# codgodtao/TMDiff

Hardware: AMD Instinct MI355X
Metric: UNet denoise-steps/sec (8-ch 64x64, batch 32) (higher is better)
Workload: dtype f32; 1 GPU; BASELINE configs[1]: batch-32 8-ch 64x64 tiles, DDPM p_sample steps of the T=1000 cosine schedule, channel_multiplier [32,64,128,256], full UNet forward (both branches) + fused DDPM update per step; batch_per_gpu=32, parallelism=batch-parallel x1, weights=key-hashed random init, text_embedding=fixed synthetic 768-d

## Files before the change

include/tmdiff_hip.h:

```cpp
#ifndef TMDIFF_HIP_H
#define TMDIFF_HIP_H

#include <stddef.h>
#include <stdint.h>

#ifdef __cplusplus
extern "C" {
#endif

#define TMDIFF_ABI_VERSION 6

#define TMDIFF_OK 0
#define TMDIFF_E_INVALID (-1)
#define TMDIFF_E_UNSUPPORTED (-2)
#define TMDIFF_E_LAUNCH (-3)

typedef void* tmdiff_stream_t;

int tmdiff_version(void);
const char* tmdiff_last_error_string(void);

typedef struct tmdiff_conv3d_desc {
  int32_t B, N, H, W;
  int32_t Cin, Cout;
// ... 15 lines not shown
  float out_scale;
  float* y;
  float* y2;
  const float* y2_shift;
  const float* y2_scale;
  int32_t y2_shift_stride, y2_scale_stride;
  int32_t y2_act;
  int32_t y2_bf16;
  int32_t x_bf16;
  void* splitk_ws;
  int64_t splitk_ws_bytes;
  uint64_t drop_seed;
  float drop_p;
  const uint64_t* drop_seed_dev;
  const float* rc_x;
  const float* rc_w;
  int32_t rc_cin;
  float* y_ll;
  float* y_hi[3];
  float* xp_out;
  const float* xp_shift;
  int32_t xp_shift_stride, xp_act;
  int32_t y2_s2d;
} tmdiff_conv3d_desc;

int tmdiff_conv3d_pack_weights(const float* w, float* packed, int32_t Cout, int32_t Cin, int32_t ksize,
                               int32_t groups, int32_t mode, tmdiff_stream_t stream);
typedef struct tmdiff_pack_entry {
  const float* w;
  float* packed_fwd;
  float* packed_dgrad;
  int32_t Cout, Cin, ksize, groups;
} tmdiff_pack_entry;
int32_t tmdiff_conv3d_pack_weights_multi_chunks(int32_t Cout, int32_t Cin, int32_t groups, int32_t* n_type_a);
int tmdiff_conv3d_pack_weights_multi(const tmdiff_pack_entry* entries_dev, const int32_t* chunk_tensor_dev,
                                     const int32_t* chunk_index_dev, int32_t n_chunks, tmdiff_stream_t stream);
int tmdiff_conv3d_fwd(const tmdiff_conv3d_desc* d, tmdiff_stream_t stream);
int tmdiff_conv3d_fwd_xp_supported(const tmdiff_conv3d_desc* d);
size_t tmdiff_conv3d_fwd_splitk_workspace_bytes(const tmdiff_conv3d_desc* d);

int tmdiff_conv3d_fwd_staged_supported(const tmdiff_conv3d_desc* d);
size_t tmdiff_conv3d_fwd_staged_workspace_bytes(const tmdiff_conv3d_desc* d);
int tmdiff_conv3d_fwd_staged(const tmdiff_conv3d_desc* d, void* workspace, tmdiff_stream_t stream);

int tmdiff_conv3d_ll_supported(const tmdiff_conv3d_desc* d);
size_t tmdiff_conv3d_ll_splitk_workspace_bytes(const tmdiff_conv3d_desc* d);
// ... 4 lines not shown

int tmdiff_conv3d_wino_supported(const tmdiff_conv3d_desc* d);
int32_t tmdiff_conv3d_wino_planes(int32_t N);
int64_t tmdiff_conv3d_wino_blocks(const tmdiff_conv3d_desc* d);
size_t tmdiff_conv3d_wino_workspace_bytes(const tmdiff_conv3d_desc* d);
size_t tmdiff_conv3d_wino_packed_bytes(int32_t Cout, int32_t Cin, int32_t groups, int32_t planes);
int tmdiff_conv3d_wino_pack_weights(const float* w, float* packed, int32_t Cout, int32_t Cin, int32_t groups,
                                    int32_t mode, int32_t planes, tmdiff_stream_t stream);
typedef struct tmdiff_wino_pack_entry {
  const float* w;
  float* packed;
  int32_t Cout, Cin, groups, mode, planes, reserved;
} tmdiff_wino_pack_entry;
int32_t tmdiff_conv3d_wino_pack_weights_multi_chunk(void);
int tmdiff_conv3d_wino_pack_weights_multi(const tmdiff_wino_pack_entry* entries_dev, const int32_t* chunk_tensor_dev,
                                          const int32_t* chunk_index_dev, int32_t n_chunks, tmdiff_stream_t stream);
int tmdiff_conv3d_wino_fwd(const tmdiff_conv3d_desc* d, void* workspace, tmdiff_stream_t stream);
int tmdiff_conv3d_wino_fwd_stage(const tmdiff_conv3d_desc* d, void* workspace, int32_t stage, tmdiff_stream_t stream);
int tmdiff_conv3d_wino_fwd_xp(const tmdiff_conv3d_desc* d, void* workspace, int32_t stage, float* xp_out, tmdiff_stream_t stream);
int tmdiff_conv3d_wino_fwd_planes(const tmdiff_conv3d_desc* d, void* workspace, int32_t stage, float* xp_out, int32_t planes,
                                  tmdiff_stream_t stream);

int tmdiff_conv3d_wf_supported(const tmdiff_conv3d_desc* d);
int64_t tmdiff_conv3d_wf_blocks(const tmdiff_conv3d_desc* d);
size_t tmdiff_conv3d_wf_splitk_workspace_bytes(const tmdiff_conv3d_desc* d);
size_t tmdiff_conv3d_wf_workspace_bytes(const tmdiff_conv3d_desc* d);
int32_t tmdiff_conv3d_wf_plan(int32_t B, int32_t Cin, int32_t Cout, int32_t N, int32_t H, int32_t W, int32_t groups, int32_t llm,
                              int64_t* tiles);
int tmdiff_conv3d_wf_fwd(const tmdiff_conv3d_desc* d, void* workspace, tmdiff_stream_t stream);
int tmdiff_conv3d_wfll_supported(const tmdiff_conv3d_desc* d);
size_t tmdiff_conv3d_wfll_packed_bytes(int32_t Cout, int32_t Cin);
int tmdiff_conv3d_wfll_pack_weights(const float* w, float* packed, int32_t Cout, int32_t Cin, float ll_scale,
                                    tmdiff_stream_t stream);
size_t tmdiff_conv3d_wfll_splitk_workspace_bytes(const tmdiff_conv3d_desc* d);
int tmdiff_conv3d_wfll_fwd(const tmdiff_conv3d_desc* d, float ll_scale, tmdiff_stream_t stream);

size_t tmdiff_conv3d_packed_bf16_bytes(int32_t Cout, int32_t Cin, int32_t ksize, int32_t groups);
int tmdiff_conv3d_pack_weights_bf16(const float* w, void* packed, int32_t Cout, int32_t Cin, int32_t ksize,
                                    int32_t groups, tmdiff_stream_t stream);
int tmdiff_conv3d_pack_weights_bf16_dgrad(const float* w, void* packed, int32_t Cout, int32_t Cin, int32_t ksize,
                                          int32_t groups, tmdiff_stream_t stream);
size_t tmdiff_conv3d_bf16_workspace_bytes(const tmdiff_conv3d_desc* d);
int tmdiff_conv3d_fwd_bf16(const tmdiff_conv3d_desc* d, void* workspace, tmdiff_stream_t stream);


int tmdiff_conv3d_prologue_fwd(const tmdiff_conv3d_desc* d, float* xp, tmdiff_stream_t stream);
// ... 259 lines not shown
```

tmdiff_amd/_lib.py:

```python
import ctypes as C
import os

_HERE = os.path.dirname(os.path.abspath(__file__))
LIB_PATH = os.environ.get("TMDIFF_HIP_LIB") or os.path.join(_HERE, "libtmdiff_hip.so")

c_float_p = C.POINTER(C.c_float)
vp = C.c_void_p


class Conv3dDesc(C.Structure):
    _fields_ = [
        ("B", C.c_int32), ("N", C.c_int32), ("H", C.c_int32), ("W", C.c_int32),
        ("Cin", C.c_int32), ("Cout", C.c_int32),
        ("groups", C.c_int32), ("ksize", C.c_int32), ("nseg", C.c_int32),
        ("seg_c", C.c_int32 * 3),
        ("seg_x", vp * 3),
        ("w_packed", vp), ("bias", vp), ("bias_scale", C.c_float),
        ("in_shift", vp), ("in_scale", vp), ("in_shift_stride", C.c_int32), ("in_scale_stride", C.c_int32),
        ("in_mask", vp), ("in_act", C.c_int32),
        ("residual", vp), ("out_scale", C.c_float),
        ("y", vp),
        ("y2", vp), ("y2_shift", vp), ("y2_scale", vp), ("y2_shift_stride", C.c_int32), ("y2_scale_stride", C.c_int32),
        ("y2_act", C.c_int32), ("y2_bf16", C.c_int32), ("x_bf16", C.c_int32),
        ("splitk_ws", vp), ("splitk_ws_bytes", C.c_int64),
        ("drop_seed", C.c_uint64), ("drop_p", C.c_float), ("drop_seed_dev", vp), ("rc_x", vp), ("rc_w", vp), ("rc_cin", C.c_int32), ("y_ll", vp), ("y_hi", vp * 3), ("xp_out", vp), ("xp_shift", vp), ("xp_shift_stride", C.c_int32), ("xp_act", C.c_int32),
        ("y2_s2d", C.c_int32),
    ]


SIGNATURES = {
    "tmdiff_version": (C.c_int, []),
    "tmdiff_last_error_string": (C.c_char_p, []),
    "tmdiff_conv3d_pack_weights": (C.c_int, [vp, vp, C.c_int32, C.c_int32, C.c_int32, C.c_int32, C.c_int32, vp]),
    "tmdiff_conv3d_pack_weights_multi_chunks": (C.c_int32, [C.c_int32, C.c_int32, C.c_int32, C.POINTER(C.c_int32)]),
    "tmdiff_conv3d_pack_weights_multi": (C.c_int, [vp, vp, vp, C.c_int32, vp]),
    "tmdiff_conv3d_fwd": (C.c_int, [C.POINTER(Conv3dDesc), vp]),
    "tmdiff_conv3d_fwd_splitk_workspace_bytes": (C.c_size_t, [C.POINTER(Conv3dDesc)]),
    "tmdiff_conv3d_fwd_xp_supported": (C.c_int, [C.POINTER(Conv3dDesc)]),
    "tmdiff_conv3d_fwd_staged_supported": (C.c_int, [C.POINTER(Conv3dDesc)]),
    "tmdiff_conv3d_fwd_staged_workspace_bytes": (C.c_size_t, [C.POINTER(Conv3dDesc)]),
    "tmdiff_conv3d_fwd_staged": (C.c_int, [C.POINTER(Conv3dDesc), vp, vp]),
    "tmdiff_conv3d_wino_supported": (C.c_int, [C.POINTER(Conv3dDesc)]),
    "tmdiff_conv3d_wino_blocks": (C.c_int64, [C.POINTER(Conv3dDesc)]),
    "tmdiff_conv3d_wino_workspace_bytes": (C.c_size_t, [C.POINTER(Conv3dDesc)]),
    "tmdiff_conv3d_wino_planes": (C.c_int32, [C.c_int32]),
    "tmdiff_conv3d_wino_packed_bytes": (C.c_size_t, [C.c_int32, C.c_int32, C.c_int32, C.c_int32]),
    "tmdiff_conv3d_wino_pack_weights": (C.c_int, [vp, vp, C.c_int32, C.c_int32, C.c_int32, C.c_int32, C.c_int32, vp]),
    "tmdiff_conv3d_wino_pack_weights_multi_chunk": (C.c_int32, []),
    "tmdiff_conv3d_wino_pack_weights_multi": (C.c_int, [vp, vp, vp, C.c_int32, vp]),
    "tmdiff_conv3d_wf_supported": (C.c_int, [C.POINTER(Conv3dDesc)]),
    "tmdiff_conv3d_wf_blocks": (C.c_int64, [C.POINTER(Conv3dDesc)]),
    "tmdiff_conv3d_wf_workspace_bytes": (C.c_size_t, [C.POINTER(Conv3dDesc)]),
    "tmdiff_conv3d_wf_splitk_workspace_bytes": (C.c_size_t, [C.POINTER(Conv3dDesc)]),
    "tmdiff_conv3d_wf_fwd": (C.c_int, [C.POINTER(Conv3dDesc), vp, vp]),
    "tmdiff_conv3d_wino_fwd": (C.c_int, [C.POINTER(Conv3dDesc), vp, vp]),
    "tmdiff_conv3d_wino_fwd_planes": (C.c_int, [C.POINTER(Conv3dDesc), vp, C.c_int32, vp, C.c_int32, vp]),
    "tmdiff_conv3d_wino_fwd_xp": (C.c_int, [C.POINTER(Conv3dDesc), vp, C.c_int32, vp, vp]),
    "tmdiff_conv3d_wino_fwd_stage": (C.c_int, [C.POINTER(Conv3dDesc), vp, C.c_int32, vp]),
    "tmdiff_conv3d_prologue_fwd": (C.c_int, [C.POINTER(Conv3dDesc), vp, vp]),
    "tmdiff_conv3d_ll_supported": (C.c_int, [C.POINTER(Conv3dDesc)]),
    "tmdiff_conv3d_ll_splitk_workspace_bytes": (C.c_size_t, [C.POINTER(Conv3dDesc)]),
    "tmdiff_conv3d_ll_packed_bytes": (C.c_size_t, [C.c_int32, C.c_int32]),
    "tmdiff_conv3d_ll_pack_weights": (C.c_int, [vp, vp, C.c_int32, C.c_int32, C.c_float, vp]),
    "tmdiff_conv3d_ll_fwd": (C.c_int, [C.POINTER(Conv3dDesc), C.c_float, vp]),
    "tmdiff_conv3d_packed_bf16_bytes": (C.c_size_t, [C.c_int32, C.c_int32, C.c_int32, C.c_int32]),
    "tmdiff_conv3d_pack_weights_bf16": (C.c_int, [vp, vp, C.c_int32, C.c_int32, C.c_int32, C.c_int32, vp]),
    "tmdiff_conv3d_bf16_workspace_bytes": (C.c_size_t, [C.POINTER(Conv3dDesc)]),
    "tmdiff_conv3d_fwd_bf16": (C.c_int, [C.POINTER(Conv3dDesc), vp, vp]),
    "tmdiff_conv3d_wgrad_workspace_bytes": (C.c_size_t, [C.POINTER(Conv3dDesc)]),
    "tmdiff_conv3d_wgrad": (C.c_int, [C.POINTER(Conv3dDesc), vp, vp, vp, vp]),
    "tmdiff_conv3d_wgrad_bias": (C.c_int, [C.POINTER(Conv3dDesc), vp, vp, vp, vp, vp]),
    "tmdiff_conv3d_wf_plan": (C.c_int32, [C.c_int32] * 8 + [C.POINTER(C.c_int64)]),
    "tmdiff_conv3d_wfll_supported": (C.c_int, [C.POINTER(Conv3dDesc)]),
    "tmdiff_conv3d_wfll_packed_bytes": (C.c_size_t, [C.c_int32, C.c_int32]),
# ... 163 lines not shown
```

tmdiff_amd/csrc/conv3d_wf.hip:

```cpp
#include <type_traits>

#include "common.h"
#include "epilogue.h"

#ifndef TMDIFF_WF_ABLATE
#define TMDIFF_WF_ABLATE 0
#endif
#ifndef TMDIFF_WF_STAMPS
#define TMDIFF_WF_STAMPS 0
#endif

namespace {

using namespace tmdiff;

using f32x4 = __attribute__((ext_vector_type(4))) float;
using f32x2 = __attribute__((ext_vector_type(2))) float;

struct WfArgs {
  int B, N, H, W;
  int Cin, Cout, cin_g, cout_g, groups;
  const float* x;
  const float* xgrp[3];
  int grouped_segs;
  const float* wp;
  const float* bias;
  float bias_scale;
  const float* residual;
  float out_scale;
  float* y;
  float* y2;
  const float* y2_shift;
  const float* y2_scale;
  int y2_shift_stride, y2_scale_stride, y2_act;
  int y2_s2d;
  int tiles_h, tiles_w, tiles_co;
  unsigned total_blocks;
  int vec4;
  int ksplit, split_chunks;
  float* part;
  unsigned long long* stamps;
  int stagger;
  unsigned first_round;
  float* yll;
  float* yhi[3];
  const float* rc_x;
  const float* rc_w;
  int rc_cin;
};

#if defined(__HIP_DEVICE_COMPILE__)
using KArgs = const WfArgs __attribute__((address_space(4)))*;
__device__ __forceinline__ KArgs kargs() {
  KArgs k = (KArgs)__builtin_amdgcn_kernarg_segment_ptr();
  asm volatile("" : "+s"(k));
  return k;
}
#else
using KArgs = const WfArgs*;
__device__ __forceinline__ KArgs kargs() { return nullptr; }
#endif

template <class T>
// ... 170 lines not shown
  using G = GeoF<TT, TH, TW, PAIR, LLM>;
  constexpr int NP = G::NP, MO = G::MO, KC = G::KC, CO = G::CO, NS = G::NS, HH = G::HH, RQ = G::RQ, PW = G::PW;
  constexpr int W_TAPS = G::W_TAPS;
  __shared__ __attribute__((aligned(16))) float lds[2 * G::STAGE + G::RAW_FLOATS];
  float* const st0 = lds;
  float* const st1 = lds + G::STAGE;
  float* const raw = lds + 2 * G::STAGE;
  static_assert(2 * G::STAGE + G::RAW_FLOATS >= 4 * 1024, "the epilogue borrows 4 KB of LDS per wave");

  const int tid = threadIdx.x;
  const int lane = tid & 63, wv = __builtin_amdgcn_readfirstlane(tid >> 6);
  const int l31 = lane & 31, khalf = lane >> 5;
#if TMDIFF_WF_STAMPS
  unsigned long long stamp_t[6];
  const unsigned long long stamp_c0 = __builtin_amdgcn_s_memtime();
  stamp_t[0] = __builtin_amdgcn_s_memrealtime();
#define WF_STAMP(i) stamp_t[i] = __builtin_amdgcn_s_memrealtime()
#else
#define WF_STAMP(i)
#endif
  stagger_start(a.stagger, a.first_round);
  WF_STAMP(1);

  unsigned id = xcd_remap(blockIdx.x, a.total_blocks);
  const int split = take(id, a.ksplit);
  const int co_tile = take(id, a.tiles_co);
  const int tw_i = take(id, a.tiles_w);
  const int th_i = take(id, a.tiles_h);
  const int g = __builtin_amdgcn_readfirstlane(id % a.groups);
  const int b = __builtin_amdgcn_readfirstlane(id / a.groups) * (PAIR ? 2 : 1);
  const bool pimg_ok = !PAIR || b + 1 < a.B;
  const int h0 = th_i * TH, w0 = tw_i * TW;
  const int co0 = co_tile * CO;
  const int hw = a.H * a.W;
  const long plane = (long)a.N * hw;
  const int nchunks = a.split_chunks;
  const float* xg = (a.grouped_segs ? (g == 0 ? a.xgrp[0] : (g == 1 ? a.xgrp[1] : a.xgrp[2])) + (long)b * a.cin_g * plane
                                    : a.x + ((long)b * a.Cin + (long)g * a.cin_g) * plane) + (long)split * nchunks * KC * plane;
  const float* wg = a.wp + ((long)g * a.cin_g + (long)split * nchunks * KC) * W_TAPS * a.cout_g + co0;

  const long xbs = PAIR && pimg_ok ? (long)(a.grouped_segs ? a.cin_g : a.Cin) * plane : 0;
  const unsigned xbytes = (unsigned)((xbs + KC * plane) * 4), wbytes = (unsigned)(KC * W_TAPS * a.cout_g * 4);
  const int xq = lane % G::REG_QUADS, xsub = lane / G::REG_QUADS;
  unsigned xlane_off;
  if constexpr (PAIR) {
    const int img = (xq % RQ) >> 1;
    xlane_off = (lane < G::PLANES && (img == 0 || pimg_ok)) ? (unsigned)((img * xbs + (xq / RQ) * hw + 4 * (xq & 1)) * 4) : buf::kOutside;
  } else {
    const int xwq = w0 - 4 + 4 * (xq % RQ);
    xlane_off = (lane < G::PLANES && xwq >= 0 && xwq < a.W) ? (unsigned)(((xq / RQ) * hw + xwq) * 4) : buf::kOutside;
  }
  auto issue_raw = [&](auto kc_, int c) __attribute__((always_inline)) {
    constexpr int k = decltype(kc_)::value;
    const int p = wv + 4 * k;
    if (G::XP % 4 == 0 || p < G::XP) {
      const buf::rsrc r = buf::make(xg + (long)c * KC * plane, xbytes);
      const int region = p * G::RPP + (G::RPP > 1 ? xsub : 0);
      const int kc = region / HH, row = region - kc * HH;
      const int h = h0 - 1 + row;
      const bool ok = h >= 0 && h < a.H && region < G::NREG;
      const unsigned lo = opaque(xlane_off);
      const unsigned voff = ok ? lo + (unsigned)((kc * (int)plane + h * a.W) * 4) : buf::kOutside;
// ... 218 lines not shown
  }
#undef WF_EPI2
#if TMDIFF_WF_STAMPS
  WF_STAMP(4);
  __builtin_amdgcn_s_waitcnt(0);
  WF_STAMP(5);
  if (a.stamps && lane == 0) {
    unsigned long long* o = a.stamps + ((unsigned long long)blockIdx.x * 4 + wv) * 8;
    for (int i = 0; i < 6; ++i) o[i] = stamp_t[i];
    o[6] = ((unsigned long long)__builtin_amdgcn_s_getreg(4 | (31 << 11)) << 32) | __builtin_amdgcn_s_getreg(6 | (31 << 11)) |
           ((unsigned long long)(__builtin_amdgcn_s_getreg(20 | (31 << 11)) & 0xf) << 28);
    o[7] = __builtin_amdgcn_s_memtime() - stamp_c0;
  }
#endif
}

template <int TT, int TH, int TW, bool PAIR = false, bool LLM = false>
int launch(WfArgs& a, hipStream_t st) {
  a.tiles_h = (a.H + TH - 1) / TH;
  a.tiles_w = PAIR ? 1 : (a.W + TW - 1) / TW;
  a.tiles_co = a.cout_g / 32;
  const long blocks = (long)a.ksplit * (PAIR ? (a.B + 1) / 2 : a.B) * a.groups * a.tiles_h * a.tiles_w * a.tiles_co;
  if (const int rc = tmdiff::set_grid(a, blocks, "conv3d_wf_fwd")) return rc;
  static const double stagger_chunks = env_double("TMDIFF_WF_STAGGER", 0.0);
  a.first_round = 512;
  a.stagger = blocks > 512 ? (int)(stagger_chunks * 2.0 * 54 * 2 * 64) : 0;
  conv3d_wf_kernel<TT, TH, TW, PAIR, LLM><<<(unsigned)blocks, 256, 0, st>>>(a);
  return tmdiff::check_launch("conv3d_wf_fwd");
}

bool wf_form_ok(const tmdiff_conv3d_desc* d) {
  if (!d || d->ksize != 3 || (d->groups != 1 && d->groups != 3) || d->in_mask || d->x_bf16 || d->y2_bf16) return false;
  if (!(d->drop_p >= 0.f && d->drop_p < 1.f)) return false;
  if (d->nseg < 1 || d->nseg > 3 || d->Cin <= 0 || d->Cout <= 0 || d->Cin % d->groups || d->Cout % d->groups) return false;
  return (d->Cin / d->groups) % 2 == 0 && (d->Cout / d->groups) % 32 == 0 && (d->N == 8 || d->N == 4) && d->H > 0 && d->W > 0 &&
         d->W % 4 == 0;
}

bool wf_grouped_segs(const tmdiff_conv3d_desc* d) {
  return d->nseg == 3 && d->groups == 3 && d->seg_c[0] == d->seg_c[1] && d->seg_c[1] == d->seg_c[2] &&
         d->seg_c[0] * 3 == d->Cin;
}

bool wf_pair(const tmdiff_conv3d_desc* d) { return d->N == 8 && d->W == 8; }

bool wf_plain(const tmdiff_conv3d_desc* d) {
// ... 15 lines not shown
  const long units = wf_pair(d) ? (d->B + 1) / 2 : (long)d->B * ((d->W + 15) / 16);
  return units * d->groups * ((d->H + th - 1) / th) * (d->Cout / d->groups / 32);
}

int wf_ksplit(const tmdiff_conv3d_desc* d, bool pairs = false) {
  static const long target = env_long("TMDIFF_SPLITK", 256);
  const long tiles = wf_tiles(d);
  const int nchunks = d->Cin / d->groups / 2;
  const int ksteps = pairs ? 24 : 54;
  if (target <= 0 || tiles <= 0) return 1;
  auto ok = [&](int s) { return s >= 1 && nchunks % s == 0 && nchunks / s >= 2 && !(pairs && (nchunks / s) % 2); };
  int best = 1;
  if (tiles < target)
    for (int s = 2; s <= nchunks / 2; ++s) {
      if (!ok(s)) continue;
      best = s;
      if (tiles * s >= target) break;
    }
  static const long long_range = env_long("TMDIFF_SPLITK_LONG", 1700);
  if (tiles * best < 384 && ok(2 * best) && (long)(nchunks / (2 * best)) * ksteps >= long_range) best *= 2;
  return best;
}

}

extern "C" int tmdiff_conv3d_wf_supported(const tmdiff_conv3d_desc* d) { return wf_shape_ok(d) ? 1 : 0; }

extern "C" int32_t tmdiff_conv3d_wf_plan(int32_t B, int32_t Cin, int32_t Cout, int32_t N, int32_t H, int32_t W, int32_t groups,
                                         int32_t llm, int64_t* tiles) {
  tmdiff_conv3d_desc d = {};
  d.B = B; d.N = N; d.H = H; d.W = W; d.Cin = Cin; d.Cout = Cout; d.groups = groups; d.ksize = 3; d.nseg = 1; d.seg_c[0] = Cin;
  if (tiles) *tiles = 0;
  if (B <= 0 || !wf_shape_ok(&d)) return 0;
  if (tiles) *tiles = wf_tiles(&d);
  return wf_ksplit(&d, llm != 0);
}

extern "C" int64_t tmdiff_conv3d_wf_blocks(const tmdiff_conv3d_desc* d) {
  if (!wf_shape_ok(d) || d->B <= 0) return 0;
  return (int64_t)wf_tiles(d) * wf_ksplit(d);
}

extern "C" size_t tmdiff_conv3d_wf_splitk_workspace_bytes(const tmdiff_conv3d_desc* d) {
  if (!wf_shape_ok(d) || d->B <= 0) return 0;
  return splitk_bytes(wf_ksplit(d), d, (long)d->N * d->H * d->W);
}

extern "C" size_t tmdiff_conv3d_wf_workspace_bytes(const tmdiff_conv3d_desc* d) {
  if (!wf_shape_ok(d) || d->B <= 0 || wf_plain(d)) return 0;
  return (size_t)d->B * d->Cin * d->N * d->H * d->W * sizeof(float);
}

namespace {
int wf_forward(const tmdiff_conv3d_desc* d, void* workspace, tmdiff_stream_t stream, bool llm, float bias_mul) {
  using namespace tmdiff;
  TMDIFF_REQUIRE(d != nullptr, "conv3d_wf_fwd: NULL descriptor");
  if (!wf_form_ok(d))
    return fail(TMDIFF_E_UNSUPPORTED, "conv3d_wf_fwd: fp32 3x3x3, groups 1 or 3, N = 8 or 4, W %% 4 == 0, Cin/g %% 2 == 0, Cout/g %% 32 == 0, no mask");
  if (!wf_fits(d))
    return fail(TMDIFF_E_UNSUPPORTED, "conv3d_wf_fwd: plane too large for 32-bit offsets (32 channels of a sample per descriptor; pair "
                                      "mode: (Cin + 2) x plane < 2^29; a prologue pass: B * Cin <= 65535)");
  TMDIFF_REQUIRE(d->B >= 0, "conv3d_wf_fwd: bad extents");
  if (d->B == 0) return TMDIFF_OK;
  TMDIFF_REQUIRE(d->w_packed && (d->y || d->y2 || d->y_ll) && aligned16(d->w_packed), "conv3d_wf_fwd: NULL / unaligned weights or output");
  const long plane = (long)d->N * d->H * d->W;
  if (const int rc = check_segments(d, "conv3d_wf_fwd", true)) return rc;
  if (!(aligned16(d->y) && aligned16(d->y2) && aligned16(d->residual)))
    return fail(TMDIFF_E_UNSUPPORTED, "conv3d_wf_fwd: 16-byte aligned outputs / residual");
  hipStream_t st = as_stream(stream);
  const float* x = d->seg_x[0];
  if (!wf_plain(d)) {
    TMDIFF_REQUIRE(workspace && aligned16(workspace), "conv3d_wf_fwd: this input needs its workspace (tmdiff_conv3d_wf_workspace_bytes)");
    const int rc = launch_prologue_apply(d, static_cast<float*>(workspace), st);
    if (rc) return rc;
    x = static_cast<const float*>(workspace);
  }
  WfArgs a;
  a.grouped_segs = wf_plain(d) && d->nseg == 3;
  for (int i = 0; i < 3; ++i) a.xgrp[i] = a.grouped_segs ? d->seg_x[i] : nullptr;
  a.B = d->B; a.N = d->N; a.H = d->H; a.W = d->W;
  a.Cin = d->Cin; a.Cout = d->Cout; a.groups = d->groups; a.cin_g = d->Cin / d->groups; a.cout_g = d->Cout / d->groups;
  a.x = x; a.wp = d->w_packed;
  set_outputs(a, d);
  a.bias_scale *= bias_mul;
  a.y2_s2d = d->y2 && d->y2_s2d ? 1 : 0;
  if (a.y2_s2d) TMDIFF_REQUIRE(d->H % 2 == 0 && d->W % 4 == 0, "conv3d_wf_fwd: the space-to-depth second output needs even H and W %% 4 == 0");
  a.vec4 = 1;
  a.stamps = TMDIFF_WF_STAMPS ? static_cast<unsigned long long*>(d->splitk_ws) : nullptr;
  a.ksplit = 1; a.split_chunks = a.cin_g / 2; a.part = nullptr;
  if (!TMDIFF_WF_STAMPS) {
    const int ks = wf_ksplit(d, llm);
    if (float* part = lend_splitk(d, ks, plane)) {
      if (a.y2_s2d)
        return fail(TMDIFF_E_UNSUPPORTED, "conv3d_wf_fwd: a grid that splits its input channels cannot write the space-to-depth second output");
      a.ksplit = ks; a.split_chunks = a.cin_g / 2 / ks; a.part = part;
    }
  }
  a.yll = nullptr; a.yhi[0] = a.yhi[1] = a.yhi[2] = nullptr;
  if (d->y_ll) {
    const bool dwt = d->y_hi[0] != nullptr;
    if (llm || wf_pair(d) || a.part || d->y || (dwt ? (d->y2 || !d->y_hi[1] || !d->y_hi[2]) : !d->y2) || d->N != 8 || d->H % 2 ||
        d->W % 4 || !aligned16(d->y_ll) || !aligned16(d->y_hi[0]) || !aligned16(d->y_hi[1]) || !aligned16(d->y_hi[2]))
      return fail(TMDIFF_E_UNSUPPORTED, "conv3d_wf_fwd: the LL / Haar output needs 8 bands, even H, W %% 4 == 0, planes wider than 8 columns, "
                                        "y == NULL (with a second output, or with all three high bands and none), and a grid that "
                                        "does not split its input channels");
    a.yll = d->y_ll;
    for (int i = 0; i < 3; ++i) a.yhi[i] = dwt ? d->y_hi[i] : nullptr;
  }
  a.rc_x = nullptr; a.rc_w = nullptr; a.rc_cin = 0;
  if (d->rc_x) {
    if (llm || wf_pair(d) || d->groups != 1 || d->residual || !d->rc_w || d->rc_cin <= 0 || d->rc_cin % 32 || d->rc_cin > 512 ||
        !aligned16(d->rc_x) || !aligned16(d->rc_w))
      return fail(TMDIFF_E_UNSUPPORTED, "conv3d_wf_fwd: a folded residual convolution needs groups 1, rc_cin %% 32 == 0 (at most 512), no residual "
                                        "tensor and planes wider than 8 columns");
    if (!wf_rc_fits(d)) return fail(TMDIFF_E_UNSUPPORTED, "conv3d_wf_fwd: rc_x sample too large for 32-bit byte offsets");
    a.rc_x = d->rc_x; a.rc_w = d->rc_w; a.rc_cin = d->rc_cin;
  }
  int rc;
// ... 60 lines not shown
extern "C" int tmdiff_conv3d_wfll_supported(const tmdiff_conv3d_desc* d) {
  tmdiff_conv3d_desc e;
  return wfll_desc(d, &e) ? 1 : 0;
}

extern "C" size_t tmdiff_conv3d_wfll_packed_bytes(int32_t Cout, int32_t Cin) {
  if (Cout <= 0 || Cin <= 0 || Cout % 32) return 0;
  return (size_t)Cin * 96 * Cout * sizeof(float);
}

extern "C" int tmdiff_conv3d_wfll_pack_weights(const float* w, float* packed, int32_t Cout, int32_t Cin, float ll_scale,
                                               tmdiff_stream_t stream) {
  using namespace tmdiff;
  TMDIFF_REQUIRE(w && packed && aligned16(packed), "conv3d_wfll_pack_weights: NULL / unaligned pointer");
  TMDIFF_REQUIRE(Cout > 0 && Cin > 0 && Cout % 32 == 0, "conv3d_wfll_pack_weights: Cout=%d (multiple of 32) Cin=%d", Cout, Cin);
  const long rows = (long)Cout * Cin;
  wfll_pack_kernel<<<(unsigned)((rows + 255) / 256), 256, 0, as_stream(stream)>>>(w, packed, Cout, Cin, ll_scale * 0.5f);
  return check_launch("conv3d_wfll_pack_weights");
}

extern "C" size_t tmdiff_conv3d_wfll_splitk_workspace_bytes(const tmdiff_conv3d_desc* d) {
  tmdiff_conv3d_desc e;
  if (!wfll_desc(d, &e) || d->B <= 0) return 0;
  return splitk_bytes(wf_ksplit(&e, true), &e, (long)e.N * e.H * e.W);
}

extern "C" int tmdiff_conv3d_wfll_fwd(const tmdiff_conv3d_desc* d, float ll_scale, tmdiff_stream_t stream) {
  using namespace tmdiff;
  tmdiff_conv3d_desc e;
  if (!wfll_desc(d, &e))
    return fail(TMDIFF_E_UNSUPPORTED, "conv3d_wfll_fwd: one plain fp32 space-to-depth input, 3x3x3, groups 1, 8 or 4 bands, even H, W %% 8 == 0, Cout %% 32 == 0");
  return wf_forward(&e, nullptr, stream, true, 2.f * ll_scale);
}
```

tmdiff_amd/ops.py:

```python
import ctypes as C
import math
import os

import numpy as np
import torch

from . import _lib, routing
from ._lib import Conv3dDesc, check, lib



class KernelConfig:

    _FLAG = lambda default: (lambda v: (v != "0") if default else (v == "1"))
    _FIELDS = {
        "winograd": ("TMDIFF_WINOGRAD", _FLAG(True), True), "wf": ("TMDIFF_WF", _FLAG(True), True),
        "wf_pair": ("TMDIFF_WF_PAIR", _FLAG(True), True), "wf_splitk": ("TMDIFF_WF_SPLITK", _FLAG(True), True),
        "wf_min_fill": ("TMDIFF_WF_MIN_FILL", float, 0.7), "wino_min_blocks": ("TMDIFF_WINO_MIN_BLOCKS", int, 256),
        "ll_compose": ("TMDIFF_LL_COMPOSE", _FLAG(True), True), "wfll": ("TMDIFF_WFLL", _FLAG(True), True),
        "train_ll_wino": ("TMDIFF_TRAIN_LL_WINO", _FLAG(True), True),
        "conv2_after_ll": ("TMDIFF_CONV2_AFTER_LL", _FLAG(True), True),
        "epilogue_fuse": ("TMDIFF_EPILOGUE_FUSE", _FLAG(True), True), "producer_fuse": ("TMDIFF_PRODUCER_FUSE", _FLAG(True), True),
        "fp32_staged": ("TMDIFF_FP32_STAGED", str, "auto"), "bf16_pack": ("TMDIFF_BF16_PACK", str, "auto"),
        "wgrad_wino": ("TMDIFF_WGRAD_WINO", _FLAG(True), True), "wgrad_wino_bias": ("TMDIFF_WGRAD_WINO_BIAS", _FLAG(True), True),
        "wgrad_bias": ("TMDIFF_WGRAD_BIAS", _FLAG(False), False), "wino_multipack": ("TMDIFF_WINO_MULTIPACK", _FLAG(True), True),
        "fuse_res_conv": ("TMDIFF_FUSE_RES_CONV", _FLAG(True), True), "emit_ll": ("TMDIFF_EMIT_LL", _FLAG(True), True),
        "emit_dwt": ("TMDIFF_EMIT_DWT", _FLAG(True), True), "side_xp": ("TMDIFF_SIDE_XP", _FLAG(True), True),
        "train_fused_resblock": ("TMDIFF_TRAIN_FUSED_RESBLOCK", _FLAG(True), True),
        "train_graph": ("TMDIFF_TRAIN_GRAPH", _FLAG(False), False),
        "train_two_streams": ("TMDIFF_TRAIN_STREAMS", _FLAG(True), True),
        "sample_graph": ("TMDIFF_SAMPLE_GRAPH", _FLAG(False), False),
        "grad_bf16": ("TMDIFF_GRAD_BF16", _FLAG(False), False),
    }

    def __init__(self, env=None):
        env = os.environ if env is None else env
        for name, (var, parse, default) in self._FIELDS.items():
            object.__setattr__(self, name, parse(env[var]) if var in env else default)

    def __setattr__(self, name, value):
# ... 413 lines not shown
        raise ValueError(f"{what}: keep_y=False needs emit=")
    return y, (torch.empty(*y2_shape, device=dev, dtype=y2_dtype) if emit is not None and y2_shape is not None else None)


def _emit_kw(emit):
    return {} if emit is None else dict(y2_act=emit.get("act", False), y2_shift=emit.get("shift"), y2_scale=emit.get("scale"),
                                        y2_shift_stride=emit.get("shift_stride", 0), y2_scale_stride=emit.get("scale_stride", 0))


def _result(y, y2):
    return y if y2 is None else ((y, y2) if y is not None else y2)


def _plain(segs, kw):
    return len(segs) == 1 and not (kw.get("in_act") or kw.get("in_shift") is not None or kw.get("in_scale") is not None or
                                   kw.get("in_mask") is not None or kw.get("drop") is not None)


def _lend_splitk(d, dev, nbytes):
    if nbytes:
        d.splitk_ws, d.splitk_ws_bytes = _workspace(dev, nbytes, "splitk").data_ptr(), nbytes


def _xp_target(what, xp_out, nbytes, dev):
    if not nbytes:
        return None
    if xp_out is None:
        return _workspace(dev, nbytes).data_ptr()
    if not (xp_out.is_cuda and xp_out.is_contiguous() and xp_out.numel() * 4 == nbytes):
        raise ValueError(f"{what}: xp_out must be a contiguous fp32 [B, Cin, N, H, W] tensor")
    return xp_out.data_ptr()


def _launch(fn, d, args, what, key, flops, ksize=3, suffix="", bytes_of=None):
    if key is not None:
        _count(key, flops)
    if TIMER is None:
        check(fn(C.byref(d), *args, stream_ptr()), what)
        return
    e0, e1 = torch.cuda.Event(enable_timing=True), torch.cuda.Event(enable_timing=True)
    e0.record()
    check(fn(C.byref(d), *args, stream_ptr()), what)
    e1.record()
    rec = (e0, e1, flops, ksize, what, _tag(d) + suffix)
    TIMER.records.append(rec if bytes_of is None else rec + (bytes_of(d),))

# ... 113 lines not shown
    b, _, n, h, w = segs[0].shape
    dev = segs[0].device
    s2d = bool(emit is not None and emit.get("s2d"))
    want_ll = bool(emit is not None and emit.get("ll"))
    want_dwt = bool(emit is not None and emit.get("dwt"))
    if want_dwt and (s2d or want_ll):
        raise ValueError("conv3d_wf: emit dwt=True excludes s2d / ll")
    want_ll = want_ll or want_dwt
    if s2d or want_ll:
        cin = sum(s_.shape[1] for s_ in segs)
        if not routing.wf_quarter_ok(b, cin, cout, n, h, w, groups):
            raise ValueError("conv3d_wf: this launch cannot write a space-to-depth / LL output (ask routing.wf_quarter_ok first)")
    if want_ll and keep_y:
        raise ValueError("conv3d_wf: the LL output replaces y (keep_y=False)")
    q = (b, cout, n, h // 2, w // 2)
    y_ll = torch.empty(*q, device=dev, dtype=torch.float32) if want_ll else None
    y_hi = [torch.empty(*q, device=dev, dtype=torch.float32) for _ in range(3)] if want_dwt else None
    y, y2 = _outputs("conv3d_wf", dev, (b, cout, n, h, w), keep_y, emit,
                     None if want_dwt else ((b, 4 * cout, n, h // 2, w // 2) if s2d else (b, cout, n, h, w)))
    d = make_conv_desc(segs, w_packed, cout, 3, y, y2=y2, groups=groups, y2_s2d=s2d, y_ll=y_ll, y_hi=y_hi, **kw,
                       **_emit_kw(emit))
    if not lib.tmdiff_conv3d_wf_supported(C.byref(d)):
        raise ValueError("conv3d_wf: shape not supported")
    _lend_splitk(d, dev, lib.tmdiff_conv3d_wf_splitk_workspace_bytes(C.byref(d)) if (config.wf_splitk and not want_ll) else 0)
    nws = lib.tmdiff_conv3d_wf_workspace_bytes(C.byref(d))
    ws = _xp_target("conv3d_wf", xp_out, nws, dev)
    if xp_out is not None and not nws:
        xp_out.copy_(segs[0] if len(segs) == 1 else torch.cat(segs, 1))
    flops = 2.0 * b * cout * ((d.Cin // groups) * 13.5 + d.rc_cin) * n * h * w
    _launch(lib.tmdiff_conv3d_wf_fwd, d, (ws,), "conv3d_wf_fwd", "conv3d_wf_fwd", flops, 3, f" +rc{d.rc_cin}" if d.rc_cin else "")
    return (y_ll, *y_hi) if want_dwt else (y2, y_ll) if want_ll else _result(y, y2)


def pack_conv_weight_ll(w, ll_scale=0.5):
    cout, cin = w.shape[0], w.shape[1]
    nb = lib.tmdiff_conv3d_ll_packed_bytes(cout, cin)
    if tuple(w.shape[2:]) != (3, 3, 3) or nb == 0:
        raise ValueError(f"pack_conv_weight_ll: weight shape {tuple(w.shape)} not supported")
    out = torch.empty(nb // 4, device=w.device, dtype=torch.float32)
    check(lib.tmdiff_conv3d_ll_pack_weights(_chk(w.detach(), "w"), out.data_ptr(), cout, cin, float(ll_scale), stream_ptr()),
          "conv3d_ll_pack_weights")
    return out


def conv3d_ll(x, w_packed, cout, ll_scale=0.5, emit=None, keep_y=True, **kw):
    b, _, n, h, w = x.shape
# ... 5 lines not shown
        raise ValueError("conv3d_ll: shape not supported (ll_conv_supported)")
    _lend_splitk(d, dev, lib.tmdiff_conv3d_ll_splitk_workspace_bytes(C.byref(d)))
    _launch(lib.tmdiff_conv3d_ll_fwd, d, (float(ll_scale),), "conv3d_ll_fwd", "conv3d_ll_fwd",
            2.0 * b * cout * d.Cin * 48 * n * (h // 2) * (w // 2))
    return _result(y, y2)


def pack_conv_weight_wfll(w, ll_scale=0.5):
    cout, cin = w.shape[0], w.shape[1]
    out = torch.empty(cin * 96 * cout, device=w.device, dtype=torch.float32)
    check(lib.tmdiff_conv3d_wfll_pack_weights(_chk(w.detach(), "w"), out.data_ptr(), cout, cin, float(ll_scale), stream_ptr()),
          "conv3d_wfll_pack_weights")
    return out


def conv3d_wf_ll(x_s2d, w_packed, cout, ll_scale=0.5, emit=None, keep_y=True, **kw):
    b, c4, n, h2, w2 = x_s2d.shape
    dev = x_s2d.device
    oshape = (b, cout, n, h2, w2)
    y, y2 = _outputs("conv3d_wf_ll", dev, oshape, keep_y, emit, oshape)
    d = make_conv_desc([x_s2d], w_packed, cout, 3, y, y2=y2, out_div=2, x_s2d=True, **kw, **_emit_kw(emit))
    if not lib.tmdiff_conv3d_wfll_supported(C.byref(d)):
        raise ValueError("conv3d_wf_ll: shape not supported")
    _lend_splitk(d, dev, lib.tmdiff_conv3d_wfll_splitk_workspace_bytes(C.byref(d)) if config.wf_splitk else 0)
    _launch(lib.tmdiff_conv3d_wfll_fwd, d, (float(ll_scale),), "conv3d_wfll_fwd", "conv3d_wfll_fwd",
            2.0 * b * cout * d.Cin * 24 * n * h2 * w2)
    return _result(y, y2)


def stem(w, bias, out_channels, xin=None, pan=None, ms=None, silu=True, out=None, out_scale=None, out_scale_stride=0,
         pack_bf16=False):
    ref = ms if ms is not None else xin
    b, n, h, wd = ref.shape
    osc = out_scale if isinstance(out_scale, int) else _chk(out_scale, "out_scale")
    if pack_bf16:
        units = torch.empty(b, out_channels // 8, n * h * wd, 8, device=ref.device, dtype=torch.int16)
        check(lib.tmdiff_stem_fwd_pack_bf16(_chk(xin, "xin"), _chk(pan, "pan"), _chk(ms, "ms"), _chk(w, "w"), _chk(bias, "bias"),
                                            osc, out_scale_stride, units.data_ptr(), b, out_channels, n, h, wd,
                                            1 if silu else 0, stream_ptr()), "stem_fwd_pack_bf16")
        return units
    y = out if out is not None else torch.empty(b, out_channels, n, h, wd, device=ref.device, dtype=torch.float32)
    osc = out_scale if isinstance(out_scale, int) else _chk(out_scale, "out_scale")
    check(lib.tmdiff_stem_fwd_scaled(_chk(xin, "xin"), _chk(pan, "pan"), _chk(ms, "ms"), _chk(w, "w"), _chk(bias, "bias"),
                                     osc, out_scale_stride, _chk(y, "y"), b, out_channels, n, h, wd, 1 if silu else 0,
                                     stream_ptr()), "stem_fwd")
    return y
# ... 949 lines not shown
```

tmdiff_amd/routing.py:

```python
import collections
import ctypes as C

from . import _lib
from ._lib import lib

PRODUCT_FAMILIES = ("wf", "wf_pair", "wfll", "ll", "staged", "fused", "bf16")
FALLBACK_FAMILIES = ("wino4", "wino2")


def _config():
    from . import ops
    return ops.config


def _grad_bf16():
    return bool(getattr(_config(), "grad_bf16", False))


def wino_weight_ok(cout, cin, ksize=3, groups=1):
    return (ksize == 3 and groups in (1, 3) and cin % groups == 0 and cout % groups == 0 and (cin // groups) % 2 == 0 and
            (cout // groups) % 32 == 0)


def staged_weight_ok(cout, cin, groups=1):
# ... 6 lines not shown


_WF_ROUTES = {}


def wf_route(b, cin, cout, n, h, w, groups=1, masked=False, llm=False):
    cfg = _config()
    key = (b, cin, cout, n, h, w, groups, masked, llm, cfg.key())
    r = _WF_ROUTES.get(key)
    if r is None:
        if len(_WF_ROUTES) > 4096:
            _WF_ROUTES.clear()
        r = _WF_ROUTES[key] = _wf_route(cfg, b, cin, cout, n, h, w, groups, masked, llm)
    return r


def _wf_route(cfg, b, cin, cout, n, h, w, groups, masked, llm):
    if cin % groups or cout % groups or masked or not cfg.wf:
        return False, 1
    tiles = C.c_int64(0)
    split = lib.tmdiff_conv3d_wf_plan(b, cin, cout, n, h, w, groups, 1 if llm else 0, C.byref(tiles))
    if split == 0:
        return False, 1
    if not cfg.wf_splitk:
        split = 1
    th = 8 if n == 8 else 16
    pair = n == 8 and w == 8
    if pair and not cfg.wf_pair:
        return False, 1
    fill = (h * w) / float(((h + th - 1) // th) * th * (8 if pair else ((w + 15) // 16) * 16))
    if pair:
        fill *= b / (2.0 * ((b + 1) // 2))
    return bool(tiles.value * split >= cfg.wino_min_blocks and fill >= cfg.wf_min_fill), split


_QUERIES = {}


def supported(query, b, cin, cout, n, h, w, groups=1, **fields):
    key = (query, b, cin, cout, n, h, w, groups, tuple(sorted(fields.items())))
    r = _QUERIES.get(key)
    if r is None:
        if len(_QUERIES) > 4096:
            _QUERIES.clear()
        seg_c = cin if isinstance(cin, tuple) else (cin,)
        d = _lib.Conv3dDesc()
        d.B, d.N, d.H, d.W, d.Cin, d.Cout, d.groups, d.ksize, d.nseg = b, n, h, w, sum(seg_c), cout, groups, 3, len(seg_c)
        for i, c in enumerate(seg_c):
            d.seg_c[i] = c
        for k, v in fields.items():
            setattr(d, k, v)
        r = _QUERIES[key] = bool(getattr(lib, query)(C.byref(d)))
    return r


def wfll_route(b, cin, cout, n, h, w):
# ... 423 lines not shown
```

Baseline: 45.34 batch32-steps/s.

## Plan uneven split-K chunk ranges for wf conv via makespan model

```diff
diff --git a/include/tmdiff_hip.h b/include/tmdiff_hip.h
--- a/include/tmdiff_hip.h
+++ b/include/tmdiff_hip.h
@@ -61,6 +61,7 @@
   const float* xp_shift;
   int32_t xp_shift_stride, xp_act;
   int32_t y2_s2d;
+  int32_t wf_ranges[8];
 } tmdiff_conv3d_desc;
 
 int tmdiff_conv3d_pack_weights(const float* w, float* packed, int32_t Cout, int32_t Cin, int32_t ksize,
@@ -111,6 +112,8 @@
                                   tmdiff_stream_t stream);
 
 int tmdiff_conv3d_wf_supported(const tmdiff_conv3d_desc* d);
+int32_t tmdiff_conv3d_wf_ranges(const tmdiff_conv3d_desc* d, int32_t llm, int32_t* first, int32_t* count, int32_t* order, int32_t cap,
+                                double* model_us);
 int64_t tmdiff_conv3d_wf_blocks(const tmdiff_conv3d_desc* d);
 size_t tmdiff_conv3d_wf_splitk_workspace_bytes(const tmdiff_conv3d_desc* d);
 size_t tmdiff_conv3d_wf_workspace_bytes(const tmdiff_conv3d_desc* d);
diff --git a/tmdiff_amd/_lib.py b/tmdiff_amd/_lib.py
--- a/tmdiff_amd/_lib.py
+++ b/tmdiff_amd/_lib.py
@@ -24,7 +24,7 @@
         ("y2_act", C.c_int32), ("y2_bf16", C.c_int32), ("x_bf16", C.c_int32),
         ("splitk_ws", vp), ("splitk_ws_bytes", C.c_int64),
         ("drop_seed", C.c_uint64), ("drop_p", C.c_float), ("drop_seed_dev", vp), ("rc_x", vp), ("rc_w", vp), ("rc_cin", C.c_int32), ("y_ll", vp), ("y_hi", vp * 3), ("xp_out", vp), ("xp_shift", vp), ("xp_shift_stride", C.c_int32), ("xp_act", C.c_int32),
-        ("y2_s2d", C.c_int32),
+        ("y2_s2d", C.c_int32), ("wf_ranges", C.c_int32 * 8),
     ]
 
 
@@ -50,6 +50,8 @@
     "tmdiff_conv3d_wino_pack_weights_multi": (C.c_int, [vp, vp, vp, C.c_int32, vp]),
     "tmdiff_conv3d_wf_supported": (C.c_int, [C.POINTER(Conv3dDesc)]),
     "tmdiff_conv3d_wf_blocks": (C.c_int64, [C.POINTER(Conv3dDesc)]),
+    "tmdiff_conv3d_wf_ranges": (C.c_int32, [C.POINTER(Conv3dDesc), C.c_int32, C.POINTER(C.c_int32), C.POINTER(C.c_int32),
+                                            C.POINTER(C.c_int32), C.c_int32, C.POINTER(C.c_double)]),
     "tmdiff_conv3d_wf_workspace_bytes": (C.c_size_t, [C.POINTER(Conv3dDesc)]),
     "tmdiff_conv3d_wf_splitk_workspace_bytes": (C.c_size_t, [C.POINTER(Conv3dDesc)]),
     "tmdiff_conv3d_wf_fwd": (C.c_int, [C.POINTER(Conv3dDesc), vp, vp]),
diff --git a/tmdiff_amd/csrc/conv3d_wf.hip b/tmdiff_amd/csrc/conv3d_wf.hip
--- a/tmdiff_amd/csrc/conv3d_wf.hip
+++ b/tmdiff_amd/csrc/conv3d_wf.hip
@@ -1,7 +1,11 @@
+#include <map>
+#include <mutex>
+#include <tuple>
 #include <type_traits>
 
 #include "common.h"
 #include "epilogue.h"
+#include "wf_plan.h"
 
 #ifndef TMDIFF_WF_ABLATE
 #define TMDIFF_WF_ABLATE 0
@@ -39,6 +43,9 @@
   int vec4;
   int ksplit, split_chunks;
   float* part;
+  unsigned tiles;
+  int rng_table;
+  int rng_first[kWfPlanMaxRanges], rng_len[kWfPlanMaxRanges], rng_split[kWfPlanMaxRanges];
   unsigned long long* stamps;
   int stagger;
   unsigned first_round;
@@ -255,8 +262,18 @@
   stagger_start(a.stagger, a.first_round);
   WF_STAMP(1);
 
-  unsigned id = xcd_remap(blockIdx.x, a.total_blocks);
-  const int split = take(id, a.ksplit);
+  unsigned id;
+  int split, first_chunk, nchunks;
+  if (a.rng_table) {
+    const KArgs ka = kargs();
+    const unsigned rslot = (unsigned)__builtin_amdgcn_readfirstlane(blockIdx.x / a.tiles);
+    id = xcd_remap(blockIdx.x - rslot * a.tiles, a.tiles);
+    split = ka->rng_split[rslot], first_chunk = ka->rng_first[rslot], nchunks = ka->rng_len[rslot];
+  } else {
+    id = xcd_remap(blockIdx.x, a.total_blocks);
+    split = take(id, a.ksplit);
+    first_chunk = split * a.split_chunks, nchunks = a.split_chunks;
+  }
   const int co_tile = take(id, a.tiles_co);
   const int tw_i = take(id, a.tiles_w);
   const int th_i = take(id, a.tiles_h);
@@ -267,10 +284,9 @@
   const int co0 = co_tile * CO;
   const int hw = a.H * a.W;
   const long plane = (long)a.N * hw;
-  const int nchunks = a.split_chunks;
   const float* xg = (a.grouped_segs ? (g == 0 ? a.xgrp[0] : (g == 1 ? a.xgrp[1] : a.xgrp[2])) + (long)b * a.cin_g * plane
-                                    : a.x + ((long)b * a.Cin + (long)g * a.cin_g) * plane) + (long)split * nchunks * KC * plane;
-  const float* wg = a.wp + ((long)g * a.cin_g + (long)split * nchunks * KC) * W_TAPS * a.cout_g + co0;
+                                    : a.x + ((long)b * a.Cin + (long)g * a.cin_g) * plane) + (long)first_chunk * KC * plane;
+  const float* wg = a.wp + ((long)g * a.cin_g + (long)first_chunk * KC) * W_TAPS * a.cout_g + co0;
 
   const long xbs = PAIR && pimg_ok ? (long)(a.grouped_segs ? a.cin_g : a.Cin) * plane : 0;
   const unsigned xbytes = (unsigned)((xbs + KC * plane) * 4), wbytes = (unsigned)(KC * W_TAPS * a.cout_g * 4);
@@ -535,6 +551,7 @@
   a.tiles_co = a.cout_g / 32;
   const long blocks = (long)a.ksplit * (PAIR ? (a.B + 1) / 2 : a.B) * a.groups * a.tiles_h * a.tiles_w * a.tiles_co;
   if (const int rc = tmdiff::set_grid(a, blocks, "conv3d_wf_fwd")) return rc;
+  a.tiles = (unsigned)(blocks / a.ksplit);
   static const double stagger_chunks = env_double("TMDIFF_WF_STAGGER", 0.0);
   a.first_round = 512;
   a.stagger = blocks > 512 ? (int)(stagger_chunks * 2.0 * 54 * 2 * 64) : 0;
@@ -596,6 +613,47 @@
   return best;
 }
 
+WfPlan wf_plan_of(const tmdiff_conv3d_desc* d, bool ll = false) {
+  static const long enabled = env_long("TMDIFF_SPLITK", 256);
+  const long tiles = wf_tiles(d);
+  const int nchunks = d->Cin / d->groups / 2;
+  WfPlan p;
+  p.chunks[0] = nchunks;
+  if (d->wf_ranges[0]) {
+    int n = 0, sum = 0;
+    bool ok = true;
+    for (; n < kWfPlanMaxRanges && d->wf_ranges[n]; ++n) {
+      p.chunks[n] = d->wf_ranges[n], sum += d->wf_ranges[n];
+      ok = ok && d->wf_ranges[n] >= 2 && !(ll && d->wf_ranges[n] % 2);
+    }
+    p.nranges = ok && sum == nchunks ? n : 0, p.table = n > 1;
+    return p;
+  }
+  if (enabled <= 0 || tiles <= 0) return p;
+  const int equal = wf_ksplit(d, ll);
+  p.nranges = equal, p.chunks[0] = nchunks / equal;
+  if (tiles * equal <= 256 || tiles * equal >= 512 || nchunks / equal < 32) return p;
+  const double out_mb = (double)d->B * d->Cout * d->N * d->H * d->W * 4.0 / 1048576.0;
+  struct Key {
+    long tiles; int nchunks; bool ll; double mb;
+    bool operator<(const Key& o) const { return std::tie(tiles, nchunks, ll, mb) < std::tie(o.tiles, o.nchunks, o.ll, o.mb); }
+  };
+  static std::mutex mu;
+  static std::map<Key, WfPlan> cache;
+  const Key key{tiles, nchunks, ll, out_mb};
+  std::lock_guard<std::mutex> lock(mu);
+  auto it = cache.find(key);
+  if (it == cache.end()) it = cache.emplace(key, wf_plan_search(WfModel{}, tiles, nchunks, ll, out_mb, equal)).first;
+  return it->second;
+}
+
+void wf_plan_ranges(const WfPlan& p, int nchunks, int32_t* first, int32_t* len, int cap) {
+  for (int j = 0, f = 0; j < p.nranges && j < cap; ++j) {
+    const int n = p.table ? p.chunks[j] : nchunks / p.nranges;
+    first[j] = f, len[j] = n, f += n;
+  }
+}
+
 }
 
 extern "C" int tmdiff_conv3d_wf_supported(const tmdiff_conv3d_desc* d) { return wf_shape_ok(d) ? 1 : 0; }
@@ -607,17 +665,17 @@
   if (tiles) *tiles = 0;
   if (B <= 0 || !wf_shape_ok(&d)) return 0;
   if (tiles) *tiles = wf_tiles(&d);
-  return wf_ksplit(&d, llm != 0);
+  return wf_plan_of(&d, llm != 0).nranges;
 }
 
 extern "C" int64_t tmdiff_conv3d_wf_blocks(const tmdiff_conv3d_desc* d) {
   if (!wf_shape_ok(d) || d->B <= 0) return 0;
-  return (int64_t)wf_tiles(d) * wf_ksplit(d);
+  return (int64_t)wf_tiles(d) * wf_plan_of(d).nranges;
 }
 
 extern "C" size_t tmdiff_conv3d_wf_splitk_workspace_bytes(const tmdiff_conv3d_desc* d) {
   if (!wf_shape_ok(d) || d->B <= 0) return 0;
-  return splitk_bytes(wf_ksplit(d), d, (long)d->N * d->H * d->W);
+  return splitk_bytes(wf_plan_of(d).nranges, d, (long)d->N * d->H * d->W);
 }
 
 extern "C" size_t tmdiff_conv3d_wf_workspace_bytes(const tmdiff_conv3d_desc* d) {
@@ -662,12 +720,26 @@
   a.vec4 = 1;
   a.stamps = TMDIFF_WF_STAMPS ? static_cast<unsigned long long*>(d->splitk_ws) : nullptr;
   a.ksplit = 1; a.split_chunks = a.cin_g / 2; a.part = nullptr;
+  a.rng_table = 0;
+  for (int j = 0; j < kWfPlanMaxRanges; ++j) a.rng_first[j] = a.rng_len[j] = a.rng_split[j] = 0;
   if (!TMDIFF_WF_STAMPS) {
-    const int ks = wf_ksplit(d, llm);
+    const WfPlan plan = wf_plan_of(d, llm);
+    if (plan.nranges == 0)
+      return fail(TMDIFF_E_INVALID, "conv3d_wf_fwd: wf_ranges must sum to Cin / groups / 2 chunks, every range of at least 2 chunks (composed-LL "
+                                    "mode: an even number)");
+    const int ks = plan.nranges;
     if (float* part = lend_splitk(d, ks, plane)) {
       if (a.y2_s2d)
         return fail(TMDIFF_E_UNSUPPORTED, "conv3d_wf_fwd: a grid that splits its input channels cannot write the space-to-depth second output");
       a.ksplit = ks; a.split_chunks = a.cin_g / 2 / ks; a.part = part;
+      if (plan.table) {
+        int32_t first[kWfPlanMaxRanges], len[kWfPlanMaxRanges];
+        int order[kWfPlanMaxRanges];
+        wf_plan_ranges(plan, a.cin_g / 2, first, len, kWfPlanMaxRanges);
+        wf_dispatch_order(plan.chunks, ks, order);
+        a.rng_table = 1;
+        for (int j = 0; j < ks; ++j) a.rng_first[j] = first[order[j]], a.rng_len[j] = len[order[j]], a.rng_split[j] = order[j];
+      }
     }
   }
   a.yll = nullptr; a.yhi[0] = a.yhi[1] = a.yhi[2] = nullptr;
@@ -774,7 +846,7 @@
 extern "C" size_t tmdiff_conv3d_wfll_splitk_workspace_bytes(const tmdiff_conv3d_desc* d) {
   tmdiff_conv3d_desc e;
   if (!wfll_desc(d, &e) || d->B <= 0) return 0;
-  return splitk_bytes(wf_ksplit(&e, true), &e, (long)e.N * e.H * e.W);
+  return splitk_bytes(wf_plan_of(&e, true).nranges, &e, (long)e.N * e.H * e.W);
 }
 
 extern "C" int tmdiff_conv3d_wfll_fwd(const tmdiff_conv3d_desc* d, float ll_scale, tmdiff_stream_t stream) {
@@ -784,3 +856,26 @@
     return fail(TMDIFF_E_UNSUPPORTED, "conv3d_wfll_fwd: one plain fp32 space-to-depth input, 3x3x3, groups 1, 8 or 4 bands, even H, W %% 8 == 0, Cout %% 32 == 0");
   return wf_forward(&e, nullptr, stream, true, 2.f * ll_scale);
 }
+
+extern "C" int32_t tmdiff_conv3d_wf_ranges(const tmdiff_conv3d_desc* d, int32_t llm, int32_t* first, int32_t* count, int32_t* order,
+                                           int32_t cap, double* model_us) {
+  tmdiff_conv3d_desc e;
+  if (llm ? !wfll_desc(d, &e) : !wf_shape_ok(d)) return 0;
+  if (!llm) e = *d;
+  if (e.B <= 0) return 0;
+  const WfPlan p = wf_plan_of(&e, llm != 0);
+  const int nchunks = e.Cin / e.groups / 2;
+  if (first && count) wf_plan_ranges(p, nchunks, first, count, cap);
+  if (order) {
+    int ord[kWfPlanMaxRanges];
+    if (p.table) wf_dispatch_order(p.chunks, p.nranges, ord);
+    for (int j = 0; j < p.nranges && j < cap; ++j) order[j] = p.table ? ord[j] : j;
+  }
+  if (model_us && p.nranges > 0) {
+    const double out_mb = (double)e.B * e.Cout * e.N * e.H * e.W * 4.0 / 1048576.0;
+    const WfModel m;
+    model_us[1] = wf_plan_model_us(m, p, wf_tiles(&e), nchunks, llm != 0, out_mb);
+    model_us[0] = model_us[1] - (p.nranges > 1 ? m.reduce_us + m.reduce_us_per_mb * (p.nranges + 1) * out_mb : 0.0);
+  }
+  return p.nranges;
+}
diff --git a/tmdiff_amd/csrc/wf_plan.h b/tmdiff_amd/csrc/wf_plan.h
--- /dev/null
+++ b/tmdiff_amd/csrc/wf_plan.h
@@ -0,0 +1,112 @@
+#pragma once
+#include <algorithm>
+#include <cmath>
+#include <vector>
+
+namespace tmdiff {
+
+constexpr int kWfPlanMaxRanges = 8;
+
+struct WfPlan {
+  int nranges = 1;
+  bool table = false;
+  int chunks[kWfPlanMaxRanges] = {};
+  double model_us = 0.0;
+};
+
+struct WfModel {
+  double chunk_pair_us = 7.42;
+  double chunk_alone_us = 4.36;
+  double ll_chunk_pair_us = 3.36, ll_chunk_alone_us = 1.98;
+  double setup_us = 2.7, partial_epilogue_us = 4.3;
+  double reduce_us = 5.5, reduce_us_per_mb = 0.145;
+  int cus = 256;
+  double margin = 0.95;
+};
+
+inline double wf_makespan(const WfModel& m, const std::vector<int>& cost, bool ll) {
+  const double pair = ll ? m.ll_chunk_pair_us : m.chunk_pair_us, alone = ll ? m.ll_chunk_alone_us : m.chunk_alone_us;
+  const double lone_speed = pair / alone, fixed = m.setup_us + m.partial_epilogue_us;
+  const int ncu = m.cus;
+  std::vector<double> w0(ncu, 0.0), w1(ncu, 0.0);
+  size_t next = 0;
+  double t = 0.0;
+  auto fill = [&]() {
+    for (int pass = 0; pass < 2 && next < cost.size(); ++pass)
+      for (int c = 0; c < ncu && next < cost.size(); ++c) {
+        const bool e0 = w0[c] <= 0.0, e1 = w1[c] <= 0.0;
+        if (pass == 0 ? (e0 && e1) : (e0 != e1)) (e0 ? w0[c] : w1[c]) = cost[next++] * pair + fixed;
+      }
+  };
+  fill();
+  for (;;) {
+    double dt = -1.0;
+    for (int c = 0; c < ncu; ++c) {
+      const bool b0 = w0[c] > 0.0, b1 = w1[c] > 0.0;
+      if (!b0 && !b1) continue;
+      const double d = b0 && b1 ? std::min(w0[c], w1[c]) : (b0 ? w0[c] : w1[c]) / lone_speed;
+      if (dt < 0.0 || d < dt) dt = d;
+    }
+    if (dt < 0.0) return t;
+    t += dt;
+    for (int c = 0; c < ncu; ++c) {
+      const bool b0 = w0[c] > 0.0, b1 = w1[c] > 0.0;
+      const double adv = b0 && b1 ? dt : dt * lone_speed;
+      if (b0 && (w0[c] -= adv) < 1e-9) w0[c] = 0.0;
+      if (b1 && (w1[c] -= adv) < 1e-9) w1[c] = 0.0;
+    }
+    fill();
+  }
+}
+
+inline void wf_dispatch_order(const int* chunks, int n, int* order) {
+  for (int i = 0; i < n; ++i) order[i] = i;
+  std::stable_sort(order, order + n, [&](int a, int b) { return chunks[a] > chunks[b]; });
+}
+
+inline double wf_plan_model_us(const WfModel& m, const WfPlan& p, long tiles, int nchunks, bool ll, double out_mb) {
+  std::vector<int> cost;
+  cost.reserve((size_t)tiles * p.nranges);
+  if (p.table) {
+    int order[kWfPlanMaxRanges];
+    wf_dispatch_order(p.chunks, p.nranges, order);
+    for (int j = 0; j < p.nranges; ++j) cost.insert(cost.end(), (size_t)tiles, p.chunks[order[j]]);
+  } else {
+    cost.assign((size_t)tiles * p.nranges, nchunks / p.nranges);
+  }
+  double us = wf_makespan(m, cost, ll);
+  if (p.nranges > 1) us += m.reduce_us + m.reduce_us_per_mb * (p.nranges + 1) * out_mb;
+  return us;
+}
+
+inline WfPlan wf_plan_search(const WfModel& m, long tiles, int nchunks, bool ll, double out_mb, int equal_split = 1,
+                             long max_blocks = 2048) {
+  WfPlan best;
+  best.nranges = equal_split, best.table = false, best.chunks[0] = nchunks / equal_split;
+  if (tiles <= 0 || nchunks < 2) return best;
+  best.model_us = wf_plan_model_us(m, best, tiles, nchunks, ll, out_mb);
+  const int unit = ll ? 2 : 1;
+  auto score = [&](const WfPlan& p) { return p.model_us * std::pow(m.margin, -std::log2((double)p.nranges)); };
+  double best_score = score(best);
+  auto consider = [&](WfPlan& p) {
+    p.model_us = wf_plan_model_us(m, p, tiles, nchunks, ll, out_mb);
+    const double sc = score(p);
+    if (sc < best_score) best = p, best_score = sc;
+  };
+  for (int R = std::max(2, equal_split); R <= kWfPlanMaxRanges && tiles * R <= max_blocks; ++R)
+    for (int a = 1; a < R; ++a)
+      for (int S = 2; S * R < nchunks; S += unit) {
+        const int rest = nchunks - (R - a) * S;
+        if (rest <= 0 || rest % a) continue;
+        const int L = rest / a;
+        if (L <= S || L % unit) continue;
+        if (L * (ll ? m.ll_chunk_alone_us : m.chunk_alone_us) >= best_score) continue;
+        WfPlan p;
+        p.nranges = R, p.table = true;
+        for (int i = 0; i < R; ++i) p.chunks[i] = i < a ? L : S;
+        consider(p);
+      }
+  return best;
+}
+
+}
diff --git a/tmdiff_amd/ops.py b/tmdiff_amd/ops.py
--- a/tmdiff_amd/ops.py
+++ b/tmdiff_amd/ops.py
@@ -16,6 +16,7 @@
     _FIELDS = {
         "winograd": ("TMDIFF_WINOGRAD", _FLAG(True), True), "wf": ("TMDIFF_WF", _FLAG(True), True),
         "wf_pair": ("TMDIFF_WF_PAIR", _FLAG(True), True), "wf_splitk": ("TMDIFF_WF_SPLITK", _FLAG(True), True),
+        "wf_ranges": ("TMDIFF_WF_RANGES", lambda v: tuple(int(x) for x in v.split(",")) if v else None, None),
         "wf_min_fill": ("TMDIFF_WF_MIN_FILL", float, 0.7), "wino_min_blocks": ("TMDIFF_WINO_MIN_BLOCKS", int, 256),
         "ll_compose": ("TMDIFF_LL_COMPOSE", _FLAG(True), True), "wfll": ("TMDIFF_WFLL", _FLAG(True), True),
         "train_ll_wino": ("TMDIFF_TRAIN_LL_WINO", _FLAG(True), True),
@@ -475,6 +476,14 @@
         d.splitk_ws, d.splitk_ws_bytes = _workspace(dev, nbytes, "splitk").data_ptr(), nbytes
 
 
+def _force_wf_ranges(d):
+    if config.wf_ranges:
+        if len(config.wf_ranges) > 8:
+            raise ValueError("ops.config.wf_ranges: at most 8 ranges")
+        for i, c in enumerate(config.wf_ranges):
+            d.wf_ranges[i] = int(c)
+
+
 def _xp_target(what, xp_out, nbytes, dev):
     if not nbytes:
         return None
@@ -634,6 +643,7 @@
                        **_emit_kw(emit))
     if not lib.tmdiff_conv3d_wf_supported(C.byref(d)):
         raise ValueError("conv3d_wf: shape not supported")
+    _force_wf_ranges(d)
     _lend_splitk(d, dev, lib.tmdiff_conv3d_wf_splitk_workspace_bytes(C.byref(d)) if (config.wf_splitk and not want_ll) else 0)
     nws = lib.tmdiff_conv3d_wf_workspace_bytes(C.byref(d))
     ws = _xp_target("conv3d_wf", xp_out, nws, dev)
@@ -685,6 +695,7 @@
     d = make_conv_desc([x_s2d], w_packed, cout, 3, y, y2=y2, out_div=2, x_s2d=True, **kw, **_emit_kw(emit))
     if not lib.tmdiff_conv3d_wfll_supported(C.byref(d)):
         raise ValueError("conv3d_wf_ll: shape not supported")
+    _force_wf_ranges(d)
     _lend_splitk(d, dev, lib.tmdiff_conv3d_wfll_splitk_workspace_bytes(C.byref(d)) if config.wf_splitk else 0)
     _launch(lib.tmdiff_conv3d_wfll_fwd, d, (float(ll_scale),), "conv3d_wfll_fwd", "conv3d_wfll_fwd",
             2.0 * b * cout * d.Cin * 24 * n * h2 * w2)
diff --git a/tmdiff_amd/routing.py b/tmdiff_amd/routing.py
--- a/tmdiff_amd/routing.py
+++ b/tmdiff_amd/routing.py
@@ -52,6 +52,8 @@
     split = lib.tmdiff_conv3d_wf_plan(b, cin, cout, n, h, w, groups, 1 if llm else 0, C.byref(tiles))
     if split == 0:
         return False, 1
+    if cfg.wf_ranges:
+        split = len(cfg.wf_ranges)
     if not cfg.wf_splitk:
         split = 1
     th = 8 if n == 8 else 16
@@ -62,6 +64,25 @@
     if pair:
         fill *= b / (2.0 * ((b + 1) // 2))
     return bool(tiles.value * split >= cfg.wino_min_blocks and fill >= cfg.wf_min_fill), split
+
+
+def wf_ranges(b, cin, cout, n, h, w, groups=1, llm=False, forced=None):
+    d = _lib.Conv3dDesc()
+    d.B, d.N, d.H, d.W, d.Cin, d.Cout, d.groups, d.ksize, d.nseg = b, n, h, w, cin, cout, groups, 3, 1
+    d.seg_c[0] = cin
+    for i, c in enumerate(forced or ()):
+        d.wf_ranges[i] = c
+    cap = 512
+    first, count, order = (C.c_int32 * cap)(), (C.c_int32 * cap)(), (C.c_int32 * cap)()
+    us = (C.c_double * 2)()
+    nr = lib.tmdiff_conv3d_wf_ranges(C.byref(d), 1 if llm else 0, first, count, order, cap, us)
+    if nr <= 0:
+        return None
+    e = (b, 4 * cin, cout, n, h // 2, w // 2) if llm else (b, cin, cout, n, h, w)
+    tiles = C.c_int64(0)
+    lib.tmdiff_conv3d_wf_plan(*e, groups, 1 if llm else 0, C.byref(tiles))
+    return dict(ranges=[(first[i], count[i]) for i in range(nr)], order=[order[i] for i in range(nr)], tiles=tiles.value,
+                makespan_us=us[0], total_us=us[1])
 
 
 _QUERIES = {}
```

Result: no change. 45.65 batch32-steps/s (median of 6 runs) (+0.7%).
